# Glaciohound/Chimera-ST

Hardware: AMD Instinct MI355X
Metric: train utterances/sec, MuST-C EN-DE s2t_transformer_m, 1/2/4/8 MI355X (higher is better)
Workload: dtype bf16

## Files before the change

chimera-st_amd/csrc/elementwise.hip:

```cpp
#include "cst_common.h"

namespace {

inline int ew_blocks(int64_t items) {
  int64_t b = cst_ceil_div(items, 256);
  return (int)(b < 1 ? 1 : (b > 4096 ? 4096 : b));
}

template <typename T>
__global__ void glu_fwd_kernel(const T* z, T* y, int64_t rows, int64_t C) {
  const int64_t cv = C / 8, total = rows * cv;
  for (int64_t i = (int64_t)blockIdx.x * blockDim.x + threadIdx.x; i < total; i += (int64_t)gridDim.x * blockDim.x) {
    const int64_t r = i / cv, c = (i % cv) * 8;
    float a[8], g[8], o[8];
    load8(z + r * 2 * C + c, a);
    load8(z + r * 2 * C + C + c, g);
#pragma unroll
    for (int e = 0; e < 8; ++e) o[e] = a[e] / (1.0f + __expf(-g[e]));
    store8(y + r * C + c, o);
  }
}

template <typename T>
__global__ void glu_bwd_kernel(const T* dy, const T* z, T* dz, int64_t rows, int64_t C) {
// ... 324 lines not shown
                             int out_dtype, const uint32_t* row_live, uint32_t epoch, cst_stream stream) {
  CST_REQUIRE(x && workspace && rows > 0 && cols > 0 && cols % 8 == 0 && ldx % 8 == 0, "cst_colsum_typed: cols/ldx must be multiples of 8");
  CST_REQUIRE((dtype == CST_F32 || dtype == CST_BF16) && (out_dtype == CST_F32 || out_dtype == CST_BF16), "cst_colsum_typed: bad dtype");
  hipStream_t s = (hipStream_t)stream;
  CstProfScope prof(CST_K_ELEMENTWISE, s, 0.0, (double)rows * cols * cst_dtype_size(dtype));
  int64_t cblocks, nchunks, rows_per;
  colsum_grid(rows, cols, cblocks, nchunks, rows_per);
  dim3 grid((unsigned)cblocks, (unsigned)nchunks);
  float* part = (float*)workspace;
  if (dtype == CST_BF16) hipLaunchKernelGGL((colsum_kernel<bf16_t, true>), grid, dim3(256), 0, s, (const bf16_t*)x, ldx, part, rows, cols, rows_per, row_live, epoch);
  else hipLaunchKernelGGL((colsum_kernel<float, true>), grid, dim3(256), 0, s, (const float*)x, ldx, part, rows, cols, rows_per, row_live, epoch);
  if (!out) return cst_check_launch("cst_colsum_typed");
  const dim3 rgrid((unsigned)cst_ceil_div(cols, 16));
  if (out_dtype == CST_BF16) hipLaunchKernelGGL(colsum_reduce_kernel<bf16_t>, rgrid, dim3(1024), 0, s, (const float*)part, (bf16_t*)out, (int)nchunks, cols);
  else hipLaunchKernelGGL(colsum_reduce_kernel<float>, rgrid, dim3(1024), 0, s, (const float*)part, (float*)out, (int)nchunks, cols);
  return cst_check_launch("cst_colsum_typed");
}

extern "C" int cst_dropout_colsum(const void* x, void* xd, void* out, void* workspace, int64_t rows, int64_t cols, int dtype, int out_dtype,
                                  float p, uint32_t key, const uint32_t* row_live, uint32_t epoch, cst_stream stream) {
  CST_REQUIRE(x && xd && workspace && rows > 0 && cols > 0 && cols % 8 == 0, "cst_dropout_colsum: cols must be a multiple of 8");
  CST_REQUIRE((dtype == CST_F32 || dtype == CST_BF16) && (out_dtype == CST_F32 || out_dtype == CST_BF16), "cst_dropout_colsum: bad dtype");
  CST_REQUIRE(p > 0.0f && p < 1.0f, "cst_dropout_colsum: p must be in (0, 1)");
  CST_REQUIRE(!row_live || epoch != 0, "cst_dropout_colsum: stamps need a non-zero epoch");
  hipStream_t s = (hipStream_t)stream;
  CstProfScope prof(CST_K_ELEMENTWISE, s, 0.0, 2.0 * (double)rows * cols * cst_dtype_size(dtype));
  int64_t cblocks, nchunks, rows_per;
  colsum_grid(rows, cols, cblocks, nchunks, rows_per);
  dim3 grid((unsigned)cblocks, (unsigned)nchunks);
  float* part = (float*)workspace;
  const uint32_t thr = cst_drop_thr16(p);
  const float scale = 1.0f / (1.0f - p);
  if (dtype == CST_BF16) hipLaunchKernelGGL((colsum_kernel<bf16_t, true, true>), grid, dim3(256), 0, s, (const bf16_t*)x, cols, part, rows, cols, rows_per, row_live, epoch, (bf16_t*)xd, key, thr, scale);
  else hipLaunchKernelGGL((colsum_kernel<float, true, true>), grid, dim3(256), 0, s, (const float*)x, cols, part, rows, cols, rows_per, row_live, epoch, (float*)xd, key, thr, scale);
  if (!out) return cst_check_launch("cst_dropout_colsum");
  const dim3 rgrid((unsigned)cst_ceil_div(cols, 16));
  if (out_dtype == CST_BF16) hipLaunchKernelGGL(colsum_reduce_kernel<bf16_t>, rgrid, dim3(1024), 0, s, (const float*)part, (bf16_t*)out, (int)nchunks, cols);
  else hipLaunchKernelGGL(colsum_reduce_kernel<float>, rgrid, dim3(1024), 0, s, (const float*)part, (float*)out, (int)nchunks, cols);
  return cst_check_launch("cst_dropout_colsum");
}

extern "C" int cst_colsum_typed(const void* x, int64_t ldx, void* out, void* workspace, int64_t rows, int64_t cols, int dtype,
                                int out_dtype, cst_stream stream) {
  return colsum_typed_impl(x, ldx, out, workspace, rows, cols, dtype, out_dtype, nullptr, 0, stream);
}

extern "C" int cst_colsum_typed_live(const void* x, int64_t ldx, void* out, void* workspace, int64_t rows, int64_t cols, int dtype,
                                     int out_dtype, const uint32_t* row_live, uint32_t epoch, cst_stream stream) {
  CST_REQUIRE(row_live && epoch != 0, "cst_colsum_typed_live: stamps / non-zero epoch required");
  return colsum_typed_impl(x, ldx, out, workspace, rows, cols, dtype, out_dtype, row_live, epoch, stream);
}

extern "C" int cst_col2im1d(const void* dcol, const void* z, void* dx, int64_t B, int64_t Lin, int64_t Lout, int64_t C, int k,
                            int stride, int pad, int dact, int dtype, cst_stream stream) {
  CST_REQUIRE(dcol && dx && B > 0 && Lin > 0 && Lout > 0 && C > 0 && C % 8 == 0 && k >= 1 && stride >= 1 && pad >= 0, "cst_col2im1d: bad args");
  CST_REQUIRE(!dact || z, "cst_col2im1d: dact needs z");
  CST_REQUIRE(dtype == CST_F32 || dtype == CST_BF16, "cst_col2im1d: bad dtype");
  hipStream_t s = (hipStream_t)stream;
  CstProfScope prof(CST_K_ELEMENTWISE, s, 0.0, ((double)B * Lout * k * C + (double)B * Lin * C * (dact ? 2.0 : 1.0)) * cst_dtype_size(dtype));
  const int blocks = ew_blocks(B * Lin * C / 8);
  if (dtype == CST_BF16) hipLaunchKernelGGL(col2im1d_kernel<bf16_t>, dim3(blocks), dim3(256), 0, s, (const bf16_t*)dcol, (const bf16_t*)z, (bf16_t*)dx, B, Lin, Lout, C, k, stride, pad, dact);
  else hipLaunchKernelGGL(col2im1d_kernel<float>, dim3(blocks), dim3(256), 0, s, (const float*)dcol, (const float*)z, (float*)dx, B, Lin, Lout, C, k, stride, pad, dact);
  return cst_check_launch("cst_col2im1d");
}

extern "C" int cst_mask_rows(const void* x, const uint8_t* mask, void* y, int64_t rows, int64_t cols, int dtype, cst_stream stream) {
  CST_REQUIRE(x && mask && y && rows > 0 && cols > 0 && cols % 8 == 0, "cst_mask_rows: bad args");
  CST_REQUIRE(dtype == CST_F32 || dtype == CST_BF16, "cst_mask_rows: bad dtype");
  hipStream_t s = (hipStream_t)stream;
  CstProfScope prof(CST_K_ELEMENTWISE, s, 0.0, 2.0 * rows * cols * cst_dtype_size(dtype));
  const int blocks = ew_blocks(rows * cols / 8);
  if (dtype == CST_BF16) hipLaunchKernelGGL(mask_rows_kernel<bf16_t>, dim3(blocks), dim3(256), 0, s, (const bf16_t*)x, mask, (bf16_t*)y, rows, cols);
  else hipLaunchKernelGGL(mask_rows_kernel<float>, dim3(blocks), dim3(256), 0, s, (const float*)x, mask, (float*)y, rows, cols);
  return cst_check_launch("cst_mask_rows");
}

extern "C" int cst_dropout(const void* x, void* y, int64_t n, float p, uint32_t key, int dtype, cst_stream stream) {
  CST_REQUIRE(x && y && n > 0 && p >= 0.0f && p < 1.0f, "cst_dropout: bad args");
  CST_REQUIRE(dtype == CST_F32 || dtype == CST_BF16, "cst_dropout: bad dtype");
  CST_REQUIRE(((uintptr_t)x % 16 == 0) && ((uintptr_t)y % 16 == 0), "cst_dropout: x/y must be 16-byte aligned");
  hipStream_t s = (hipStream_t)stream;
  CstProfScope prof(CST_K_ELEMENTWISE, s, 0.0, 2.0 * n * cst_dtype_size(dtype));
  const int blocks = ew_blocks(cst_ceil_div(n, 8));
  const uint32_t thr = cst_drop_thr16(p);
  const float scale = 1.0f / (1.0f - p);
  if (dtype == CST_BF16) hipLaunchKernelGGL(dropout_kernel<bf16_t>, dim3(blocks), dim3(256), 0, s, (const bf16_t*)x, (bf16_t*)y, n, key, thr, scale);
  else hipLaunchKernelGGL(dropout_kernel<float>, dim3(blocks), dim3(256), 0, s, (const float*)x, (float*)y, n, key, thr, scale);
  return cst_check_launch("cst_dropout");
}


extern "C" int cst_rows_pack(const void* src, const int32_t* seq_off, void* dst, int64_t B, int64_t T, int64_t C, int tail_sum, int dtype,
                             cst_stream stream) {
  CST_REQUIRE(src && seq_off && dst && B > 0 && T > 0 && C > 0, "cst_rows_pack: bad args");
  CST_REQUIRE(dtype == CST_F32 || dtype == CST_BF16, "cst_rows_pack: bad dtype %d", dtype);
  CST_REQUIRE(C % 8 == 0 && B < 65536, "cst_rows_pack: C=%lld must be a multiple of 8", (long long)C);
  hipStream_t s = (hipStream_t)stream;
  CstProfScope prof(CST_K_ELEMENTWISE, s, 0.0, 2.0 * B * T * C * cst_dtype_size(dtype));
  const dim3 grid((unsigned)cst_ceil_div(T, 4), (unsigned)B);
  if (dtype == CST_BF16) hipLaunchKernelGGL(rows_pack_kernel<bf16_t>, grid, dim3(256), 0, s, (const bf16_t*)src, seq_off, (bf16_t*)dst, (int)T, (int)C, tail_sum);
  else hipLaunchKernelGGL(rows_pack_kernel<float>, grid, dim3(256), 0, s, (const float*)src, seq_off, (float*)dst, (int)T, (int)C, tail_sum);
  return cst_check_launch("cst_rows_pack");
}

extern "C" int cst_rows_unpack(const void* src, const int32_t* seq_off, void* dst, int64_t B, int64_t T, int64_t C, int tail_broadcast, int dtype,
                               cst_stream stream) {
  CST_REQUIRE(src && seq_off && dst && B > 0 && T > 0 && C > 0, "cst_rows_unpack: bad args");
  CST_REQUIRE(dtype == CST_F32 || dtype == CST_BF16, "cst_rows_unpack: bad dtype %d", dtype);
  CST_REQUIRE(C % 8 == 0 && B < 65536, "cst_rows_unpack: C=%lld must be a multiple of 8", (long long)C);
  hipStream_t s = (hipStream_t)stream;
  CstProfScope prof(CST_K_ELEMENTWISE, s, 0.0, 2.0 * B * T * C * cst_dtype_size(dtype));
  const dim3 grid((unsigned)cst_ceil_div(T, 4), (unsigned)B);
  if (dtype == CST_BF16) hipLaunchKernelGGL(rows_unpack_kernel<bf16_t>, grid, dim3(256), 0, s, (const bf16_t*)src, seq_off, (bf16_t*)dst, (int)T, (int)C, tail_broadcast);
  else hipLaunchKernelGGL(rows_unpack_kernel<float>, grid, dim3(256), 0, s, (const float*)src, seq_off, (float*)dst, (int)T, (int)C, tail_broadcast);
  return cst_check_launch("cst_rows_unpack");
}

namespace {
constexpr int WN_ROWS = 256;

template <typename T, bool DOT>
__global__ __launch_bounds__(256) void wn_partial_kernel(const T* v, const T* dw, float* part, int64_t R, int C) {
  const int gpr = C / 8, rl = threadIdx.x / gpr, cg = threadIdx.x % gpr, rpp = 256 / gpr;
  __shared__ float red[256 * 8];
  float acc[8] = {0, 0, 0, 0, 0, 0, 0, 0};
  const int64_t r0 = (int64_t)blockIdx.x * WN_ROWS;
  if (rl < rpp)
    for (int64_t r = r0 + rl; r < r0 + WN_ROWS && r < R; r += rpp) {
      float a[8], b[8];
      load8(v + r * C + cg * 8, a);
      if (DOT) load8(dw + r * C + cg * 8, b);
#pragma unroll
      for (int e = 0; e < 8; ++e) acc[e] += DOT ? a[e] * b[e] : a[e] * a[e];
    }
#pragma unroll
  for (int e = 0; e < 8; ++e) red[threadIdx.x * 8 + e] = acc[e];
  __syncthreads();
  if ((int)threadIdx.x < C) {
    const int c = threadIdx.x, g8 = c / 8, e = c % 8;
    float s = 0.0f;
    for (int l = 0; l < rpp; ++l) s += red[(l * gpr + g8) * 8 + e];
    part[(int64_t)blockIdx.x * C + c] = s;
  }
}

template <typename T>
__global__ __launch_bounds__(256) void wn_apply_fwd_kernel(const T* v, const T* g, T* w, float* norm, const float* part, int nchunks, int64_t R, int C) {
  __shared__ float scale[256];
  if ((int)threadIdx.x < C) {
    float s = 0.0f;
    for (int k = 0; k < nchunks; ++k) s += part[(int64_t)k * C + threadIdx.x];
    const float n = sqrtf(s);
    if (blockIdx.x == 0) norm[threadIdx.x] = n;
    scale[threadIdx.x] = DT<T>::ld(g + threadIdx.x) / n;
  }
  __syncthreads();
  const int gpr = C / 8;
  const int64_t total = R * gpr;
  for (int64_t i = (int64_t)blockIdx.x * 256 + threadIdx.x; i < total; i += (int64_t)gridDim.x * 256) {
    const int cg = (int)(i % gpr);
    float a[8];
    load8(v + i * 8, a);
#pragma unroll
    for (int e = 0; e < 8; ++e) a[e] *= scale[cg * 8 + e];
    store8(w + i * 8, a);
  }
}

template <typename T>
__global__ __launch_bounds__(256) void wn_apply_bwd_kernel(const T* v, const T* g, const T* dw, const float* norm, T* dv, T* dg, const float* part,
                                                           int nchunks, int64_t R, int C) {
  __shared__ float sc[256], co[256];
  if ((int)threadIdx.x < C) {
    float dot = 0.0f;
    for (int k = 0; k < nchunks; ++k) dot += part[(int64_t)k * C + threadIdx.x];
    const float n = norm[threadIdx.x], gg = DT<T>::ld(g + threadIdx.x);
    sc[threadIdx.x] = gg / n;
    co[threadIdx.x] = dot / (n * n);
    if (blockIdx.x == 0) DT<T>::st(dg + threadIdx.x, dot / n);
  }
  __syncthreads();
  const int gpr = C / 8;
  const int64_t total = R * gpr;
  for (int64_t i = (int64_t)blockIdx.x * 256 + threadIdx.x; i < total; i += (int64_t)gridDim.x * 256) {
    const int cg = (int)(i % gpr);
    float a[8], b[8];
    load8(v + i * 8, a);
    load8(dw + i * 8, b);
#pragma unroll
    for (int e = 0; e < 8; ++e) a[e] = sc[cg * 8 + e] * (b[e] - a[e] * co[cg * 8 + e]);
    store8(dv + i * 8, a);
  }
}
}

extern "C" int64_t cst_weight_norm_workspace(int64_t R, int64_t C) { return cst_ceil_div(R, WN_ROWS) * C * (int64_t)sizeof(float); }

extern "C" int cst_weight_norm_fwd(const void* v, const void* g, void* w, float* norm, void* workspace, int64_t R, int64_t C, int dtype,
                                   cst_stream stream) {
  CST_REQUIRE(v && g && w && norm && workspace && R > 0, "cst_weight_norm_fwd: null tensor");
  CST_REQUIRE(C % 8 == 0 && C >= 8 && C <= 256 && 256 % (C / 8) == 0, "cst_weight_norm_fwd: C = %lld (need a multiple of 8 up to 256 whose eighth divides 256)", (long long)C);
  hipStream_t s = (hipStream_t)stream;
  CstProfScope prof(CST_K_ELEMENTWISE, s, 0.0, (double)R * C * cst_dtype_size(dtype) * 3);
  const int nch = (int)cst_ceil_div(R, WN_ROWS);
  const int blocks = (int)(cst_ceil_div(R * (C / 8), 256) < 1024 ? cst_ceil_div(R * (C / 8), 256) : 1024);
  if (dtype == CST_BF16) {
    hipLaunchKernelGGL((wn_partial_kernel<bf16_t, false>), dim3(nch), dim3(256), 0, s, (const bf16_t*)v, (const bf16_t*)nullptr, (float*)workspace, R, (int)C);
    hipLaunchKernelGGL(wn_apply_fwd_kernel<bf16_t>, dim3(blocks), dim3(256), 0, s, (const bf16_t*)v, (const bf16_t*)g, (bf16_t*)w, norm, (const float*)workspace, nch, R, (int)C);
  } else {
    hipLaunchKernelGGL((wn_partial_kernel<float, false>), dim3(nch), dim3(256), 0, s, (const float*)v, (const float*)nullptr, (float*)workspace, R, (int)C);
    hipLaunchKernelGGL(wn_apply_fwd_kernel<float>, dim3(blocks), dim3(256), 0, s, (const float*)v, (const float*)g, (float*)w, norm, (const float*)workspace, nch, R, (int)C);
  }
  return cst_check_launch("cst_weight_norm_fwd");
}

extern "C" int cst_weight_norm_bwd(const void* v, const void* g, const void* dw, const float* norm, void* dv, void* dg, void* workspace, int64_t R,
                                   int64_t C, int dtype, cst_stream stream) {
  CST_REQUIRE(v && g && dw && norm && dv && dg && workspace && R > 0, "cst_weight_norm_bwd: null tensor");
  CST_REQUIRE(C % 8 == 0 && C >= 8 && C <= 256 && 256 % (C / 8) == 0, "cst_weight_norm_bwd: C = %lld", (long long)C);
  hipStream_t s = (hipStream_t)stream;
  CstProfScope prof(CST_K_ELEMENTWISE, s, 0.0, (double)R * C * cst_dtype_size(dtype) * 5);
  const int nch = (int)cst_ceil_div(R, WN_ROWS);
  const int blocks = (int)(cst_ceil_div(R * (C / 8), 256) < 1024 ? cst_ceil_div(R * (C / 8), 256) : 1024);
  if (dtype == CST_BF16) {
    hipLaunchKernelGGL((wn_partial_kernel<bf16_t, true>), dim3(nch), dim3(256), 0, s, (const bf16_t*)v, (const bf16_t*)dw, (float*)workspace, R, (int)C);
    hipLaunchKernelGGL(wn_apply_bwd_kernel<bf16_t>, dim3(blocks), dim3(256), 0, s, (const bf16_t*)v, (const bf16_t*)g, (const bf16_t*)dw, norm, (bf16_t*)dv, (bf16_t*)dg,
                       (const float*)workspace, nch, R, (int)C);
  } else {
    hipLaunchKernelGGL((wn_partial_kernel<float, true>), dim3(nch), dim3(256), 0, s, (const float*)v, (const float*)dw, (float*)workspace, R, (int)C);
    hipLaunchKernelGGL(wn_apply_bwd_kernel<float>, dim3(blocks), dim3(256), 0, s, (const float*)v, (const float*)g, (const float*)dw, norm, (float*)dv, (float*)dg,
                       (const float*)workspace, nch, R, (int)C);
  }
  return cst_check_launch("cst_weight_norm_bwd");
}

namespace {
template <typename T>
__device__ __forceinline__ void transpose_tile(const T* src, T* dst, int64_t R, int64_t C, int64_t r0, int64_t c0, T* tile) {
  constexpr int V = DT<T>::VEC, TS = 64, LDT = TS + V;
  constexpr int VPR = TS / V;
  for (int v = threadIdx.x; v < TS * VPR; v += 256) {
    const int r = v / VPR, cv = (v % VPR) * V;
    u32x4 x = {0, 0, 0, 0};
    if (r0 + r < R && c0 + cv < C) x = *reinterpret_cast<const u32x4*>(src + (r0 + r) * C + c0 + cv);
    *reinterpret_cast<u32x4*>(tile + r * LDT + cv) = x;
  }
  __syncthreads();
  for (int v = threadIdx.x; v < TS * VPR; v += 256) {
    const int c = v / VPR, rv = (v % VPR) * V;
    if (c0 + c < C && r0 + rv < R) {
      T out[V];
#pragma unroll
      for (int e = 0; e < V; ++e) out[e] = tile[(rv + e) * LDT + c];
      *reinterpret_cast<u32x4*>(dst + (c0 + c) * R + r0 + rv) = *reinterpret_cast<const u32x4*>(out);
    }
  }
}

template <typename T>
__global__ __launch_bounds__(256) void transpose2d_kernel(const T* src, T* dst, int64_t R, int64_t C) {
  __shared__ __attribute__((aligned(16))) T tile[64 * (64 + DT<T>::VEC)];
  transpose_tile<T>(src, dst, R, C, (int64_t)blockIdx.y * 64, (int64_t)blockIdx.x * 64, tile);
}

template <typename T>
__global__ __launch_bounds__(256) void transpose2d_multi_kernel(const cst_transpose_item* items, int n) {
  __shared__ __attribute__((aligned(16))) T tile[64 * (64 + DT<T>::VEC)];
  const int64_t b = blockIdx.x;
  int lo = 0, hi = n - 1;
  while (lo < hi) {
    const int mid = (lo + hi + 1) >> 1;
    if (items[mid].tile0 <= b) lo = mid; else hi = mid - 1;
  }
  const cst_transpose_item it = items[lo];
  const int64_t t = b - it.tile0, tx = (it.C + 63) / 64;
  transpose_tile<T>((const T*)it.src, (T*)it.dst, it.R, it.C, (t / tx) * 64, (t % tx) * 64, tile);
}
}

extern "C" int cst_transpose2d_multi(const cst_transpose_item* items_dev, int n, int64_t total_tiles, int dtype, cst_stream stream) {
  CST_REQUIRE(items_dev && n > 0 && total_tiles > 0 && total_tiles < (1ll << 31), "cst_transpose2d_multi: bad table");
  CST_REQUIRE(dtype == CST_F32 || dtype == CST_BF16, "cst_transpose2d_multi: bad dtype");
  hipStream_t s = (hipStream_t)stream;
  CstProfScope prof(CST_K_ELEMENTWISE, s, 0.0, 2.0 * (double)total_tiles * 4096 * cst_dtype_size(dtype));
  if (dtype == CST_BF16) hipLaunchKernelGGL(transpose2d_multi_kernel<bf16_t>, dim3((unsigned)total_tiles), dim3(256), 0, s, items_dev, n);
  else hipLaunchKernelGGL(transpose2d_multi_kernel<float>, dim3((unsigned)total_tiles), dim3(256), 0, s, items_dev, n);
  return cst_check_launch("cst_transpose2d_multi");
}

namespace {
struct ReduceTable { cst_reduce_item it[CST_REDUCE_MAX_ITEMS]; int n; };

__global__ __launch_bounds__(1024) void reduce_multi_kernel(ReduceTable t) {
  __shared__ float ra[64][65];
  const int b = blockIdx.x;
  int lo = 0, hi = t.n - 1;
  while (lo < hi) {
    const int mid = (lo + hi + 1) >> 1;
    if (t.it[mid].block0 <= b) lo = mid; else hi = mid - 1;
  }
  const cst_reduce_item& it = t.it[lo];
  const int64_t blk = b - it.block0;
  if (it.order == 0) {
    const int64_t i0 = (blk * 1024 + threadIdx.x) * 8;
    if (i0 >= it.L) return;
    const float* src = it.src + i0;
    float v[8] = {0.0f, 0.0f, 0.0f, 0.0f, 0.0f, 0.0f, 0.0f, 0.0f};
    int sp = 0;
    for (; sp + 4 <= it.P; sp += 4) {
      f32x4 a[4][2];
#pragma unroll
      for (int u = 0; u < 4; ++u) {
        a[u][0] = *reinterpret_cast<const f32x4*>(src + (int64_t)(sp + u) * it.stride);
        a[u][1] = *reinterpret_cast<const f32x4*>(src + (int64_t)(sp + u) * it.stride + 4);
      }
#pragma unroll
      for (int u = 0; u < 4; ++u)
#pragma unroll
        for (int e = 0; e < 4; ++e) { v[e] += a[u][0][e]; v[4 + e] += a[u][1][e]; }
    }
    for (; sp < it.P; ++sp) {
      const f32x4 a0 = *reinterpret_cast<const f32x4*>(src + (int64_t)sp * it.stride), a1 = *reinterpret_cast<const f32x4*>(src + (int64_t)sp * it.stride + 4);
#pragma unroll
      for (int e = 0; e < 4; ++e) { v[e] += a0[e]; v[4 + e] += a1[e]; }
    }
    if (it.dst_dtype == CST_BF16) store8((bf16_t*)it.dst + i0, v);
    else store8((float*)it.dst + i0, v);
    return;
  }
  const int cl = threadIdx.x & 15, g = threadIdx.x >> 4;
  const int64_t c = blk * 64 + cl * 4;
  f32x4 a = {0.0f, 0.0f, 0.0f, 0.0f};
  if (c < it.L) {
    const float* src = it.src + c;
    int i = g;
    for (; i + 192 < it.P; i += 256) {
      const f32x4 v0 = *reinterpret_cast<const f32x4*>(src + (int64_t)i * it.stride), v1 = *reinterpret_cast<const f32x4*>(src + (int64_t)(i + 64) * it.stride);
      const f32x4 v2 = *reinterpret_cast<const f32x4*>(src + (int64_t)(i + 128) * it.stride), v3 = *reinterpret_cast<const f32x4*>(src + (int64_t)(i + 192) * it.stride);
#pragma unroll
      for (int e = 0; e < 4; ++e) a[e] = (((a[e] + v0[e]) + v1[e]) + v2[e]) + v3[e];
    }
    for (; i < it.P; i += 64) {
      const f32x4 v = *reinterpret_cast<const f32x4*>(src + (int64_t)i * it.stride);
#pragma unroll
      for (int e = 0; e < 4; ++e) a[e] += v[e];
    }
  }
#pragma unroll
  for (int e = 0; e < 4; ++e) ra[g][cl * 4 + e] = a[e];
  __syncthreads();
  if (threadIdx.x < 64) {
    const int64_t cc = blk * 64 + threadIdx.x;
    if (cc < it.L) {
      float t = ra[0][threadIdx.x];
#pragma unroll 8
      for (int k = 1; k < 64; ++k) t += ra[k][threadIdx.x];
      if (it.dst_dtype == CST_BF16) DT<bf16_t>::st((bf16_t*)it.dst + cc, t);
      else ((float*)it.dst)[cc] = t;
    }
  }
}
}

extern "C" int cst_reduce_multi(const cst_reduce_item* items, int n, cst_stream stream) {
  CST_REQUIRE(items && n > 0 && n <= CST_REDUCE_MAX_ITEMS, "cst_reduce_multi: 1..%d items per call", CST_REDUCE_MAX_ITEMS);
  ReduceTable t;
  int64_t blocks = 0;
  double bytes = 0.0;
  for (int i = 0; i < n; ++i) {
    const cst_reduce_item& it = items[i];
    CST_REQUIRE(it.src && it.dst && it.L > 0 && it.L % 8 == 0 && it.P > 0 && it.stride % 4 == 0 && ((uintptr_t)it.src % 16) == 0 && ((uintptr_t)it.dst % 16) == 0,
                "cst_reduce_multi: item %d: L, stride, alignment", i);
    CST_REQUIRE((it.dst_dtype == CST_F32 || it.dst_dtype == CST_BF16) && (it.order == 0 || it.order == 1), "cst_reduce_multi: item %d: bad dst_dtype / order", i);
    t.it[i] = it;
    t.it[i].block0 = (int32_t)blocks;
    blocks += it.order == 0 ? cst_ceil_div(it.L, 8192) : cst_ceil_div(it.L, 64);
    bytes += (double)it.L * ((double)it.P * 4.0 + cst_dtype_size(it.dst_dtype));
  }
  CST_REQUIRE(blocks < (1ll << 31), "cst_reduce_multi: too many blocks");
  t.n = n;
  hipStream_t s = (hipStream_t)stream;
  CstProfScope prof(CST_K_ELEMENTWISE, s, 0.0, bytes);
  hipLaunchKernelGGL(reduce_multi_kernel, dim3((unsigned)blocks), dim3(1024), 0, s, t);
  return cst_check_launch("cst_reduce_multi");
}

extern "C" int cst_transpose2d(const void* src, void* dst, int64_t R, int64_t C, int dtype, cst_stream stream) {
  CST_REQUIRE(src && dst && R > 0 && C > 0, "cst_transpose2d: null tensor");
  const int v = dtype == CST_BF16 ? 8 : 4;
  CST_REQUIRE(R % v == 0 && C % v == 0, "cst_transpose2d: R and C must be multiples of %d", v);
  hipStream_t s = (hipStream_t)stream;
  CstProfScope prof(CST_K_ELEMENTWISE, s, 0.0, 2.0 * (double)R * C * cst_dtype_size(dtype));
  dim3 grid((unsigned)cst_ceil_div(C, 64), (unsigned)cst_ceil_div(R, 64));
  if (dtype == CST_BF16) hipLaunchKernelGGL(transpose2d_kernel<bf16_t>, grid, dim3(256), 0, s, (const bf16_t*)src, (bf16_t*)dst, R, C);
  else hipLaunchKernelGGL(transpose2d_kernel<float>, grid, dim3(256), 0, s, (const float*)src, (float*)dst, R, C);
  return cst_check_launch("cst_transpose2d");
}
```

chimera-st_amd/csrc/layernorm.hip:

```cpp
#include "cst_common.h"

namespace {

constexpr int LN_MAXV = 4;
constexpr int LN_WAVES = 4;

template <typename T> struct Raw8;
template <> struct Raw8<bf16_t> {
  u32x4 r;
  __device__ __forceinline__ void load(const bf16_t* p) { r = *reinterpret_cast<const u32x4*>(p); }
  __device__ __forceinline__ void unpack(float (&v)[8]) const {
#pragma unroll
    for (int i = 0; i < 4; ++i) { v[2 * i] = __uint_as_float(r[i] << 16); v[2 * i + 1] = __uint_as_float(r[i] & 0xffff0000u); }
  }
};
template <> struct Raw8<float> {
  float f[8];
  __device__ __forceinline__ void load(const float* p) { load8(p, f); }
  __device__ __forceinline__ void unpack(float (&v)[8]) const {
#pragma unroll
    for (int i = 0; i < 8; ++i) v[i] = f[i];
  }
};

template <typename T, int NV>
__global__ __launch_bounds__(LN_WAVES * 64) void ln_fwd_kernel(const T* x, const T* res, const T* gamma, const T* beta,
                                                              T* y, T* sum_out, float* mean, float* rstd,
                                                              int64_t rows, int cols, float eps) {
  const int lane = threadIdx.x & 63, wave = threadIdx.x >> 6;
  const int nvec = cols / 8;
  Raw8<T> gq[NV], bq[NV], nx[NV], nr[NV];
#pragma unroll
  for (int i = 0; i < NV; ++i)
    if (lane + 64 * i < nvec) { gq[i].load(gamma + (lane + 64 * i) * 8); bq[i].load(beta + (lane + 64 * i) * 8); }
  const int64_t row0 = (int64_t)blockIdx.x * LN_WAVES + wave, rstep = (int64_t)gridDim.x * LN_WAVES;
  if (row0 < rows) {
#pragma unroll
    for (int i = 0; i < NV; ++i)
      if (lane + 64 * i < nvec) {
        nx[i].load(x + row0 * cols + (lane + 64 * i) * 8);
        if (res) nr[i].load(res + row0 * cols + (lane + 64 * i) * 8);
      }
  }
  for (int64_t row = row0; row < rows; row += rstep) {
    float v[NV][8];
    float s = 0.0f;
#pragma unroll
    for (int i = 0; i < NV; ++i) {
      const int vi = lane + 64 * i;
      if (vi < nvec) {
        nx[i].unpack(v[i]);
        if (res) {
          float r[8];
          nr[i].unpack(r);
#pragma unroll
          for (int e = 0; e < 8; ++e) v[i][e] += r[e];
        }
      }
    }
    if (row + rstep < rows) {
#pragma unroll
      for (int i = 0; i < NV; ++i)
        if (lane + 64 * i < nvec) {
          nx[i].load(x + (row + rstep) * cols + (lane + 64 * i) * 8);
          if (res) nr[i].load(res + (row + rstep) * cols + (lane + 64 * i) * 8);
        }
    }
#pragma unroll
    for (int i = 0; i < NV; ++i) {
      const int vi = lane + 64 * i;
      if (vi < nvec) {
        if (sum_out) store8(sum_out + row * cols + vi * 8, v[i]);
#pragma unroll
        for (int e = 0; e < 8; ++e) s += v[i][e];
      }
    }
    const float mu = wave_sum(s) / (float)cols;
    float q = 0.0f;
#pragma unroll
    for (int i = 0; i < NV; ++i)
      if (lane + 64 * i < nvec) {
#pragma unroll
        for (int e = 0; e < 8; ++e) { const float d = v[i][e] - mu; q += d * d; }
      }
    const float rs = rsqrtf(wave_sum(q) / (float)cols + eps);
#pragma unroll
    for (int i = 0; i < NV; ++i) {
      const int vi = lane + 64 * i;
      if (vi < nvec) {
        float g[8], b[8], o[8];
        gq[i].unpack(g);
        bq[i].unpack(b);
#pragma unroll
        for (int e = 0; e < 8; ++e) o[e] = (v[i][e] - mu) * rs * g[e] + b[e];
        store8(y + row * cols + vi * 8, o);
      }
    }
    if (lane == 0) { mean[row] = mu; rstd[row] = rs; }
  }
}

template <typename T, int NV>
__global__ __launch_bounds__(LN_WAVES * 64, (NV <= 2 ? 4 : 2)) void ln_bwd_kernel(const T* dy, const T* s, const T* gamma, const float* mean,
                                                              const float* rstd, const T* dres, T* dx, float* part,
                                                              int64_t rows, int cols, uint32_t* tile_live, uint32_t epoch) {
  __shared__ float red[LN_WAVES][64 * 8];
  const int lane = threadIdx.x & 63, wave = threadIdx.x >> 6;
  const int nvec = cols / 8;
  float dg[NV][8], db[NV][8], gm[NV][8];
#pragma unroll
  for (int i = 0; i < NV; ++i) {
#pragma unroll
    for (int e = 0; e < 8; ++e) { dg[i][e] = 0.0f; db[i][e] = 0.0f; gm[i][e] = 0.0f; }
    if (lane + 64 * i < nvec) load8(gamma + (lane + 64 * i) * 8, gm[i]);
  }
  for (int64_t row = (int64_t)blockIdx.x * LN_WAVES + wave; row < rows; row += (int64_t)gridDim.x * LN_WAVES) {
    const float mu = mean[row], rs = rstd[row];
    Raw8<T> rd[NV], rx[NV];
    float s1 = 0.0f, s2 = 0.0f;
#pragma unroll
    for (int i = 0; i < NV; ++i) {
      const int vi = lane + 64 * i;
      if (vi < nvec) {
        rd[i].load(dy + row * cols + vi * 8);
        rx[i].load(s + row * cols + vi * 8);
        float d[8], xs[8];
        rd[i].unpack(d);
        rx[i].unpack(xs);
#pragma unroll
        for (int e = 0; e < 8; ++e) {
          const float xh = (xs[e] - mu) * rs;
          const float g = d[e] * gm[i][e];
          s1 += g;
          s2 += g * xh;
          dg[i][e] += d[e] * xh;
          db[i][e] += d[e];
        }
      }
    }
    s1 = wave_sum(s1) / (float)cols;
    s2 = wave_sum(s2) / (float)cols;
    bool nz = false;
#pragma unroll
    for (int i = 0; i < NV; ++i) {
      const int vi = lane + 64 * i;
      if (vi < nvec) {
        float d[8], xs[8], o[8];
        rd[i].unpack(d);
        rx[i].unpack(xs);
#pragma unroll
        for (int e = 0; e < 8; ++e) o[e] = rs * (d[e] * gm[i][e] - s1 - (xs[e] - mu) * rs * s2);
        if (dres) {
          float r[8];
          load8(dres + row * cols + vi * 8, r);
#pragma unroll
          for (int e = 0; e < 8; ++e) o[e] += r[e];
        }
#pragma unroll
        for (int e = 0; e < 8; ++e) nz |= (o[e] != 0.0f);
        store8(dx + row * cols + vi * 8, o);
      }
    }
    if (tile_live && __builtin_amdgcn_ballot_w64(nz) != 0 && lane == 0) tile_live[row >> 6] = epoch;
  }
  float* pg = part + (int64_t)blockIdx.x * 2 * cols;
  float* pb = pg + cols;
#pragma unroll
  for (int i = 0; i < NV; ++i) {
    for (int pass = 0; pass < 2; ++pass) {
      __syncthreads();
#pragma unroll
      for (int e = 0; e < 8; ++e) red[wave][lane * 8 + e] = pass ? db[i][e] : dg[i][e];
      __syncthreads();
      if (wave == 0 && lane + 64 * i < nvec) {
#pragma unroll
        for (int e = 0; e < 8; ++e) {
          float a = 0.0f;
#pragma unroll
          for (int w = 0; w < LN_WAVES; ++w) a += red[w][lane * 8 + e];
          (pass ? pb : pg)[(lane + 64 * i) * 8 + e] = a;
        }
      }
    }
  }
}

template <typename TO>
__global__ __launch_bounds__(1024) void ln_bwd_reduce_kernel(const float* part, TO* dgamma, TO* dbeta, int nblocks, int cols) {
  __shared__ float ra[64][17], rb[64][17];
  const int cl = threadIdx.x & 15, g = threadIdx.x >> 4;
  const int c = blockIdx.x * 16 + cl;
  float a = 0.0f, b = 0.0f;
  if (c < cols)
    for (int i = g; i < nblocks; i += 64) {
      a += part[(int64_t)i * 2 * cols + c];
      b += part[(int64_t)i * 2 * cols + cols + c];
    }
  ra[g][cl] = a;
  rb[g][cl] = b;
  __syncthreads();
  if (g == 0 && c < cols) {
#pragma unroll 8
    for (int k = 1; k < 64; ++k) { a += ra[k][cl]; b += rb[k][cl]; }
    DT<TO>::st(dgamma + c, a);
    DT<TO>::st(dbeta + c, b);
  }
}

int ln_blocks(int64_t rows, int cap = 1024) {
  int64_t b = cst_ceil_div(rows, LN_WAVES);
  return (int)(b < cap ? b : cap);
}
inline int ln_nv(int64_t cols) { return cols <= 512 ? 1 : (cols <= 1024 ? 2 : 4); }

}

extern "C" int cst_layernorm_fwd(const void* x, const void* res, const void* gamma, const void* beta, void* y,
                                 void* sum_out, float* mean, float* rstd, int64_t rows, int64_t cols, float eps,
                                 int dtype, cst_stream stream) {
  CST_REQUIRE(x && gamma && beta && y && mean && rstd, "cst_layernorm_fwd: null tensor");
  CST_REQUIRE(rows > 0 && cols > 0 && cols % 8 == 0 && cols <= 8 * 64 * LN_MAXV, "cst_layernorm_fwd: cols=%lld must be a multiple of 8 and <= %d", (long long)cols, 8 * 64 * LN_MAXV);
  hipStream_t s = (hipStream_t)stream;
  const double bytes = (double)rows * cols * cst_dtype_size(dtype) * (2.0 + (res ? 1.0 : 0.0) + (sum_out ? 1.0 : 0.0));
  CstProfScope prof(CST_K_LAYERNORM, s, 0.0, bytes);
  dim3 grid(ln_blocks(rows, 2048));
  CST_REQUIRE(dtype == CST_BF16 || dtype == CST_F32, "cst_layernorm_fwd: bad dtype %d", dtype);
#define CST_LNF(T, NVV) hipLaunchKernelGGL((ln_fwd_kernel<T, NVV>), grid, dim3(LN_WAVES * 64), 0, s, (const T*)x, (const T*)res, (const T*)gamma, (const T*)beta, (T*)y, (T*)sum_out, mean, rstd, rows, (int)cols, eps)
#define CST_LNF_NV(T) do { const int nv = ln_nv(cols); if (nv == 1) CST_LNF(T, 1); else if (nv == 2) CST_LNF(T, 2); else CST_LNF(T, 4); } while (0)
  if (dtype == CST_BF16) CST_LNF_NV(bf16_t);
  else CST_LNF_NV(float);
#undef CST_LNF_NV
#undef CST_LNF
  return cst_check_launch("cst_layernorm_fwd");
}

constexpr int LN_BWD_BLOCKS = 1024;
extern "C" int64_t cst_layernorm_bwd_workspace(int64_t rows, int64_t cols) {
  return (int64_t)ln_blocks(rows, LN_BWD_BLOCKS) * 2 * cols * (int64_t)sizeof(float);
}

static int layernorm_bwd_impl(const void* dy, const void* sx, const void* gamma, const float* mean, const float* rstd,
                              const void* dres, void* dx, void* dgamma, void* dbeta, void* workspace, int64_t rows,
                              int64_t cols, int dtype, int grad_dtype, uint32_t* tile_live, uint32_t epoch, cst_stream stream) {
  CST_REQUIRE(dy && sx && gamma && mean && rstd && dx && workspace && ((dgamma != nullptr) == (dbeta != nullptr)), "cst_layernorm_bwd: null tensor");
  CST_REQUIRE(rows > 0 && cols > 0 && cols % 8 == 0 && cols <= 8 * 64 * LN_MAXV, "cst_layernorm_bwd: cols=%lld must be a multiple of 8 and <= %d", (long long)cols, 8 * 64 * LN_MAXV);
  hipStream_t s = (hipStream_t)stream;
  const double bytes = (double)rows * cols * cst_dtype_size(dtype) * (3.0 + (dres ? 1.0 : 0.0));
  CstProfScope prof(CST_K_LAYERNORM, s, 0.0, bytes);
  const int nb = ln_blocks(rows, LN_BWD_BLOCKS);
  CST_REQUIRE(dtype == CST_BF16 || dtype == CST_F32, "cst_layernorm_bwd: bad dtype %d", dtype);
#define CST_LNB(T, NVV) hipLaunchKernelGGL((ln_bwd_kernel<T, NVV>), dim3(nb), dim3(LN_WAVES * 64), 0, s, (const T*)dy, (const T*)sx, (const T*)gamma, mean, rstd, (const T*)dres, (T*)dx, (float*)workspace, rows, (int)cols, tile_live, epoch)
#define CST_LNB_NV(T) do { const int nv = ln_nv(cols); if (nv == 1) CST_LNB(T, 1); else if (nv == 2) CST_LNB(T, 2); else CST_LNB(T, 4); } while (0)
  if (dtype == CST_BF16) CST_LNB_NV(bf16_t);
  else CST_LNB_NV(float);
#undef CST_LNB_NV
#undef CST_LNB
  int rc = cst_check_launch("cst_layernorm_bwd");
  if (rc != CST_OK) return rc;
  CST_REQUIRE(grad_dtype == CST_F32 || grad_dtype == dtype, "cst_layernorm_bwd: grad_dtype must be f32 or dtype");
  if (!dgamma) return rc;
  if (grad_dtype == CST_BF16)
    hipLaunchKernelGGL(ln_bwd_reduce_kernel<bf16_t>, dim3((unsigned)cst_ceil_div(cols, 16)), dim3(1024), 0, s, (const float*)workspace, (bf16_t*)dgamma, (bf16_t*)dbeta, nb, (int)cols);
  else
    hipLaunchKernelGGL(ln_bwd_reduce_kernel<float>, dim3((unsigned)cst_ceil_div(cols, 16)), dim3(1024), 0, s, (const float*)workspace, (float*)dgamma, (float*)dbeta, nb, (int)cols);
  return cst_check_launch("cst_layernorm_bwd reduce");
}

extern "C" int cst_layernorm_bwd(const void* dy, const void* sx, const void* gamma, const float* mean, const float* rstd,
                                 const void* dres, void* dx, void* dgamma, void* dbeta, void* workspace, int64_t rows,
                                 int64_t cols, int dtype, int grad_dtype, cst_stream stream) {
  return layernorm_bwd_impl(dy, sx, gamma, mean, rstd, dres, dx, dgamma, dbeta, workspace, rows, cols, dtype, grad_dtype, nullptr, 0, stream);
}

extern "C" int cst_layernorm_bwd_tiles(const void* dy, const void* sx, const void* gamma, const float* mean, const float* rstd,
                                       const void* dres, void* dx, void* dgamma, void* dbeta, void* workspace, int64_t rows,
                                       int64_t cols, int dtype, int grad_dtype, uint32_t* tile_live, uint32_t epoch, cst_stream stream) {
  CST_REQUIRE(tile_live && epoch != 0, "cst_layernorm_bwd_tiles: tile_live / non-zero epoch required");
  return layernorm_bwd_impl(dy, sx, gamma, mean, rstd, dres, dx, dgamma, dbeta, workspace, rows, cols, dtype, grad_dtype, tile_live, epoch, stream);
}
```

Baseline: 498.2.

## Prefetch next row in LayerNorm backward and narrow per-thread width in reduce

The LayerNorm backward kernel now software-pipelines its row loop for bf16 with NV>=2: it loads dy, s and dres for the next row while computing the current one. Gamma stays packed as raw bf16 in registers, and inline-asm pins keep the loaded values in VGPRs. The order-0 reduction now handles 4 floats per thread instead of 8, with an 8-deep unrolled load loop and twice as many blocks, to raise memory-level parallelism. Explicit FMA and contraction-off helpers pin down the rounding of the dx math. The prefetch raises register pressure and may lower occupancy.

After: 498.5, median of 3. Within noise of the previous version (+0.1%).

```diff
diff --git a/chimera-st_amd/csrc/elementwise.hip b/chimera-st_amd/csrc/elementwise.hip
--- a/chimera-st_amd/csrc/elementwise.hip
+++ b/chimera-st_amd/csrc/elementwise.hip
@@ -650,30 +650,43 @@
   const cst_reduce_item& it = t.it[lo];
   const int64_t blk = b - it.block0;
   if (it.order == 0) {
-    const int64_t i0 = (blk * 1024 + threadIdx.x) * 8;
+    const int64_t i0 = (blk * 1024 + threadIdx.x) * 4;
     if (i0 >= it.L) return;
     const float* src = it.src + i0;
-    float v[8] = {0.0f, 0.0f, 0.0f, 0.0f, 0.0f, 0.0f, 0.0f, 0.0f};
+    f32x4 v = {0.0f, 0.0f, 0.0f, 0.0f};
     int sp = 0;
+    for (; sp + 8 <= it.P; sp += 8) {
+      f32x4 a[8];
+#pragma unroll
+      for (int u = 0; u < 8; ++u) a[u] = *reinterpret_cast<const f32x4*>(src + (int64_t)(sp + u) * it.stride);
+#pragma unroll
+      for (int u = 0; u < 8; ++u)
+#pragma unroll
+        for (int e = 0; e < 4; ++e) v[e] += a[u][e];
+    }
     for (; sp + 4 <= it.P; sp += 4) {
-      f32x4 a[4][2];
-#pragma unroll
-      for (int u = 0; u < 4; ++u) {
-        a[u][0] = *reinterpret_cast<const f32x4*>(src + (int64_t)(sp + u) * it.stride);
-        a[u][1] = *reinterpret_cast<const f32x4*>(src + (int64_t)(sp + u) * it.stride + 4);
-      }
+      f32x4 a[4];
+#pragma unroll
+      for (int u = 0; u < 4; ++u) a[u] = *reinterpret_cast<const f32x4*>(src + (int64_t)(sp + u) * it.stride);
 #pragma unroll
       for (int u = 0; u < 4; ++u)
 #pragma unroll
-        for (int e = 0; e < 4; ++e) { v[e] += a[u][0][e]; v[4 + e] += a[u][1][e]; }
+        for (int e = 0; e < 4; ++e) v[e] += a[u][e];
     }
     for (; sp < it.P; ++sp) {
-      const f32x4 a0 = *reinterpret_cast<const f32x4*>(src + (int64_t)sp * it.stride), a1 = *reinterpret_cast<const f32x4*>(src + (int64_t)sp * it.stride + 4);
-#pragma unroll
-      for (int e = 0; e < 4; ++e) { v[e] += a0[e]; v[4 + e] += a1[e]; }
-    }
-    if (it.dst_dtype == CST_BF16) store8((bf16_t*)it.dst + i0, v);
-    else store8((float*)it.dst + i0, v);
+      const f32x4 a0 = *reinterpret_cast<const f32x4*>(src + (int64_t)sp * it.stride);
+#pragma unroll
+      for (int e = 0; e < 4; ++e) v[e] += a0[e];
+    }
+    if (it.dst_dtype == CST_BF16) {
+      typedef __bf16 bf16x4_t __attribute__((ext_vector_type(4)));
+      bf16x4_t o;
+#pragma unroll
+      for (int e = 0; e < 4; ++e) o[e] = static_cast<__bf16>(v[e]);
+      *reinterpret_cast<bf16x4_t*>((bf16_t*)it.dst + i0) = o;
+    } else {
+      *reinterpret_cast<f32x4*>((float*)it.dst + i0) = v;
+    }
     return;
   }
   const int cl = threadIdx.x & 15, g = threadIdx.x >> 4;
@@ -722,7 +735,7 @@
     CST_REQUIRE((it.dst_dtype == CST_F32 || it.dst_dtype == CST_BF16) && (it.order == 0 || it.order == 1), "cst_reduce_multi: item %d: bad dst_dtype / order", i);
     t.it[i] = it;
     t.it[i].block0 = (int32_t)blocks;
-    blocks += it.order == 0 ? cst_ceil_div(it.L, 8192) : cst_ceil_div(it.L, 64);
+    blocks += it.order == 0 ? cst_ceil_div(it.L, 4096) : cst_ceil_div(it.L, 64);
     bytes += (double)it.L * ((double)it.P * 4.0 + cst_dtype_size(it.dst_dtype));
   }
   CST_REQUIRE(blocks < (1ll << 31), "cst_reduce_multi: too many blocks");
diff --git a/chimera-st_amd/csrc/layernorm.hip b/chimera-st_amd/csrc/layernorm.hip
--- a/chimera-st_amd/csrc/layernorm.hip
+++ b/chimera-st_amd/csrc/layernorm.hip
@@ -9,6 +9,7 @@
 template <> struct Raw8<bf16_t> {
   u32x4 r;
   __device__ __forceinline__ void load(const bf16_t* p) { r = *reinterpret_cast<const u32x4*>(p); }
+  __device__ __forceinline__ void pin() { asm volatile("" : "+v"(r)); }
   __device__ __forceinline__ void unpack(float (&v)[8]) const {
 #pragma unroll
     for (int i = 0; i < 4; ++i) { v[2 * i] = __uint_as_float(r[i] << 16); v[2 * i + 1] = __uint_as_float(r[i] & 0xffff0000u); }
@@ -17,6 +18,7 @@
 template <> struct Raw8<float> {
   float f[8];
   __device__ __forceinline__ void load(const float* p) { load8(p, f); }
+  __device__ __forceinline__ void pin() {}
   __device__ __forceinline__ void unpack(float (&v)[8]) const {
 #pragma unroll
     for (int i = 0; i < 8; ++i) v[i] = f[i];
@@ -100,42 +102,98 @@
   }
 }
 
+__device__ __forceinline__ void ln_bwd_stats(float d, float xs, float gm, float mu, float rs, float& s1, float& s2, float& dg, float& db) {
+#pragma clang fp contract(off)
+  const float xh = (xs - mu) * rs;
+  const float g = d * gm;
+  s1 += g;
+  s2 += g * xh;
+  dg = __builtin_fmaf(d, xh, dg);
+  db += d;
+}
+template <int FORM>
+__device__ __forceinline__ float ln_bwd_dx(float d, float xs, float gm, float mu, float rs, float s1, float s2) {
+#pragma clang fp contract(off)
+  const float xh = (xs - mu) * rs;
+  float t;
+  if constexpr (FORM == 2) t = d * gm - s1;
+  else t = __builtin_fmaf(d, gm, -s1);
+  if constexpr (FORM == 0) t = __builtin_fmaf(-s2, xh, t);
+  else t = t - s2 * xh;
+  return rs * t;
+}
+
 template <typename T, int NV>
 __global__ __launch_bounds__(LN_WAVES * 64, (NV <= 2 ? 4 : 2)) void ln_bwd_kernel(const T* dy, const T* s, const T* gamma, const float* mean,
                                                               const float* rstd, const T* dres, T* dx, float* part,
                                                               int64_t rows, int cols, uint32_t* tile_live, uint32_t epoch) {
   __shared__ float red[LN_WAVES][64 * 8];
-  const int lane = threadIdx.x & 63, wave = threadIdx.x >> 6;
+  const int lane = threadIdx.x & 63, wave = __builtin_amdgcn_readfirstlane(threadIdx.x >> 6);
   const int nvec = cols / 8;
-  float dg[NV][8], db[NV][8], gm[NV][8];
+  float dg[NV][8], db[NV][8];
+  Raw8<T> gq[NV];
 #pragma unroll
   for (int i = 0; i < NV; ++i) {
 #pragma unroll
-    for (int e = 0; e < 8; ++e) { dg[i][e] = 0.0f; db[i][e] = 0.0f; gm[i][e] = 0.0f; }
-    if (lane + 64 * i < nvec) load8(gamma + (lane + 64 * i) * 8, gm[i]);
-  }
-  for (int64_t row = (int64_t)blockIdx.x * LN_WAVES + wave; row < rows; row += (int64_t)gridDim.x * LN_WAVES) {
-    const float mu = mean[row], rs = rstd[row];
-    Raw8<T> rd[NV], rx[NV];
+    for (int e = 0; e < 8; ++e) { dg[i][e] = 0.0f; db[i][e] = 0.0f; }
+    if (lane + 64 * i < nvec) gq[i].load(gamma + (lane + 64 * i) * 8);
+  }
+  constexpr bool PIPE = sizeof(T) == 2 && NV >= 2;
+  const int64_t row0 = (int64_t)blockIdx.x * LN_WAVES + wave, rstep = (int64_t)gridDim.x * LN_WAVES;
+  Raw8<T> nd[NV], nx[NV], nr[NV];
+  float nmu = 0.0f, nrs = 0.0f;
+  if (PIPE && row0 < rows) {
+    nmu = mean[row0];
+    nrs = rstd[row0];
+#pragma unroll
+    for (int i = 0; i < NV; ++i)
+      if (lane + 64 * i < nvec) {
+        nd[i].load(dy + row0 * cols + (lane + 64 * i) * 8);
+        nx[i].load(s + row0 * cols + (lane + 64 * i) * 8);
+        if (dres) nr[i].load(dres + row0 * cols + (lane + 64 * i) * 8);
+      }
+  }
+  for (int64_t row = row0; row < rows; row += rstep) {
+    Raw8<T> rd[NV], rx[NV], rr[NV];
+    float mu, rs;
+    if constexpr (PIPE) {
+      mu = nmu;
+      rs = nrs;
+#pragma unroll
+      for (int i = 0; i < NV; ++i) { rd[i] = nd[i]; rx[i] = nx[i]; rr[i] = nr[i]; }
+      if (row + rstep < rows) {
+        nmu = mean[row + rstep];
+        nrs = rstd[row + rstep];
+#pragma unroll
+        for (int i = 0; i < NV; ++i)
+          if (lane + 64 * i < nvec) {
+            nd[i].load(dy + (row + rstep) * cols + (lane + 64 * i) * 8);
+            nx[i].load(s + (row + rstep) * cols + (lane + 64 * i) * 8);
+            if (dres) nr[i].load(dres + (row + rstep) * cols + (lane + 64 * i) * 8);
+          }
+      }
+    } else {
+      mu = mean[row];
+      rs = rstd[row];
+#pragma unroll
+      for (int i = 0; i < NV; ++i)
+        if (lane + 64 * i < nvec) {
+          rd[i].load(dy + row * cols + (lane + 64 * i) * 8);
+          rx[i].load(s + row * cols + (lane + 64 * i) * 8);
+        }
+    }
     float s1 = 0.0f, s2 = 0.0f;
 #pragma unroll
     for (int i = 0; i < NV; ++i) {
       const int vi = lane + 64 * i;
       if (vi < nvec) {
-        rd[i].load(dy + row * cols + vi * 8);
-        rx[i].load(s + row * cols + vi * 8);
-        float d[8], xs[8];
+        float d[8], xs[8], gm[8];
+        rd[i].pin(); rx[i].pin(); gq[i].pin();
         rd[i].unpack(d);
         rx[i].unpack(xs);
-#pragma unroll
-        for (int e = 0; e < 8; ++e) {
-          const float xh = (xs[e] - mu) * rs;
-          const float g = d[e] * gm[i][e];
-          s1 += g;
-          s2 += g * xh;
-          dg[i][e] += d[e] * xh;
-          db[i][e] += d[e];
-        }
+        gq[i].unpack(gm);
+#pragma unroll
+        for (int e = 0; e < 8; ++e) ln_bwd_stats(d[e], xs[e], gm[e], mu, rs, s1, s2, dg[i][e], db[i][e]);
       }
     }
     s1 = wave_sum(s1) / (float)cols;
@@ -145,14 +203,19 @@
     for (int i = 0; i < NV; ++i) {
       const int vi = lane + 64 * i;
       if (vi < nvec) {
-        float d[8], xs[8], o[8];
+        float d[8], xs[8], gm[8], o[8];
+        rd[i].pin(); rx[i].pin(); gq[i].pin();
         rd[i].unpack(d);
         rx[i].unpack(xs);
-#pragma unroll
-        for (int e = 0; e < 8; ++e) o[e] = rs * (d[e] * gm[i][e] - s1 - (xs[e] - mu) * rs * s2);
+        gq[i].unpack(gm);
+#pragma unroll
+        for (int e = 0; e < 6; ++e) o[e] = ln_bwd_dx<0>(d[e], xs[e], gm[e], mu, rs, s1, s2);
+        o[6] = ln_bwd_dx<NV == 1 ? 1 : 0>(d[6], xs[6], gm[6], mu, rs, s1, s2);
+        o[7] = ln_bwd_dx<NV == 1 ? 2 : 0>(d[7], xs[7], gm[7], mu, rs, s1, s2);
         if (dres) {
           float r[8];
-          load8(dres + row * cols + vi * 8, r);
+          if constexpr (PIPE) { rr[i].pin(); rr[i].unpack(r); }
+          else load8(dres + row * cols + vi * 8, r);
 #pragma unroll
           for (int e = 0; e < 8; ++e) o[e] += r[e];
         }
```
